# utiasASRL/dICP

Measured on AMD Instinct MI355X. Metric: ICP cloud-iterations/sec (fwd+bwd), B=256x16384-pt clouds per GPU, higher is better.
Workload: dtype f32

## Files before the change

### dicp_amd/_lib.py

```python
import ctypes
import os
import subprocess
import threading

_HERE = os.path.dirname(os.path.abspath(__file__))
_ROOT = os.path.dirname(_HERE)
LIB_PATH = os.environ.get("DICP_HIP_LIB") or os.path.join(_HERE, "libdicp_hip.so")
SOURCES = [os.path.join(_HERE, "csrc", f) for f in ("dicp_kernels.hip", "knn_f16.hip", "dicp_call.hip", "normals.hip", "voxel.hip", "knn_points.hip", "fps.hip", "ball_query.hip", "knn_grid.hip", "group.hip", "inverse.hip", "knn_det.hip", "normals_det.hip", "filter.hip")]
HEADERS = ([os.path.join(_HERE, "csrc", f) for f in ("dicp_math.h", "dicp_common.h", "dicp_internal.h", "dicp_fill.h", "dicp_normals.h", "dicp_voxel.h", "dicp_topk.h", "dicp_fps.h", "dicp_ball.h", "dicp_gridknn.h", "kernels_grid.h", "kernels_grid_plan.h", "dicp_group.h", "dicp_group_launch.h", "dicp_inverse.h", "dicp_knn_det.h", "kernels_normals.h", "dicp_normals_det.h", "dicp_filter.h")]
           + [os.path.join(_HERE, "csrc", "kernels_%s.h" % f) for f in ("setup", "search", "setup_sort", "rows", "accumulate", "backward", "soft_svd", "host")]
           + [os.path.join(_ROOT, "include", "dicp_hip.h")])

F32, F64 = 0, 1
PT2PT, PT2PL = 0, 1
LOSS_NONE, LOSS_HUBER, LOSS_CAUCHY, LOSS_TRIM = 0, 1, 2, 3
KNN_AUTO, KNN_VALU, KNN_MFMA, KNN_SWEEP, KNN_GUMBEL = 0, 1, 2, 3, 4
FPS_AUTO, FPS_RESIDENT, FPS_STREAMED = 0, 1, 2
POOL_SUM, POOL_MEAN, POOL_MAX = 0, 1, 2
NACC_PAD, NBWD_PAD, KAB_SAVE = 32, 16, 40
PAIR_SHARDS = 64
ABI_VERSION = 11
_ERRORS = {1: "null pointer", 2: "bad shape/stride", 3: "unsupported dtype", 4: "bad enum value", 5: "misaligned buffer"}

vp, i32, i64, f64 = ctypes.c_void_p, ctypes.c_int32, ctypes.c_int64, ctypes.c_double
# ... 152 lines not shown
    "dicp_accumulate_bwd_window": ([i32, ctypes.POINTER(WeightParams), vp, vp, i32, vp, vp, vp, vp, vp, vp, vp, vp, vp, i32, i32, i32, vp, vp, vp, vp, vp, i32, vp], ctypes.c_int),
    "dicp_resolve_matches": ([vp, vp, i32, vp, i32, i32, vp, vp], ctypes.c_int),
    "dicp_match_order_scratch_bytes": ([i32, i32, i32], ctypes.c_size_t),
    "dicp_match_order": ([i32, vp, vp, i32, i32, vp, ctypes.c_size_t, vp, vp], ctypes.c_int),
    "dicp_window_reduce": ([i32, vp, vp, vp, vp, vp, vp, i32, i32, i32, i32, i32, vp, i32, i32, vp], ctypes.c_int),
    "dicp_permute_add_rows": ([i32, vp, vp, i32, i32, i32, i32, i32, i32, vp, i32, i32, vp], ctypes.c_int),
    "dicp_pose_grad_in": ([i32, vp, vp, i32, vp], ctypes.c_int),
    "dicp_pose_grad_out": ([i32, vp, vp, i32, vp, i32, vp], ctypes.c_int),
    "dicp_permute_rows": ([i32, vp, vp, i32, i32, i32, i32, i32, i32, vp, i32, i32, vp], ctypes.c_int),
    "dicp_gather_rows": ([i32, vp, vp, i32, i32, i32, i32, vp, vp], ctypes.c_int),
    "dicp_scatter_add_rows": ([i32, vp, vp, i32, i32, i32, i32, vp, vp], ctypes.c_int),
    "dicp_pack_list": ([i32, vp, vp, vp, i32, i32, i32, vp, vp, vp], ctypes.c_int),
    "dicp_unpack_list": ([i32, vp, vp, vp, vp, i32, i32, i32, i32, vp], ctypes.c_int),
    "dicp_accumulate": ([i32, ctypes.POINTER(WeightParams), vp, vp, i32, vp, vp, vp, vp, vp, i32, i32, i32, vp, vp, i64, vp], ctypes.c_int),
    "dicp_step": ([i32, ctypes.POINTER(StepIO), i32, vp], ctypes.c_int),
    "dicp_icp_forward": ([i32, ctypes.POINTER(WeightParams), ctypes.POINTER(LoopBuffers), i32, i32, i32, i32, i32, f64, i32, i32, vp], ctypes.c_int),
    "dicp_icp_forward_plan": ([i32, ctypes.POINTER(WeightParams), ctypes.POINTER(LoopBuffers), ctypes.POINTER(SegmentPlan), i32, i32, i32, i32, i32, f64, vp], ctypes.c_int),
    "dicp_icp_backward": ([i32, ctypes.POINTER(WeightParams), ctypes.POINTER(LoopBuffers), i32, i32, i32, i32, vp, vp, i32, vp, vp, vp, vp, vp, vp, i32, i32, vp], ctypes.c_int),
    "dicp_step_bwd": ([i32, vp, vp, i32, i32, vp, vp, i64, vp, vp, vp, vp, i32, vp], ctypes.c_int),
    "dicp_accumulate_bwd": ([i32, ctypes.POINTER(WeightParams), vp, vp, i32, vp, vp, vp, vp, vp, vp, vp, i32, i32, i32, vp, vp, vp, vp, vp], ctypes.c_int),
    "dicp_gumbel_nn": ([i32, vp, vp, i32, vp, ctypes.c_uint32, f64, f64, i32, i32, i32, vp, vp, vp], ctypes.c_int),
    "dicp_gumbel_nn_bwd": ([i32, vp, vp, i32, vp, ctypes.c_uint32, f64, f64, vp, vp, vp, i32, i32, i32, vp, vp, vp], ctypes.c_int),
    "dicp_kabsch_accumulate": ([i32, vp, vp, i32, vp, vp, vp, i32, f64, vp, i32, i32, i32, vp, vp], ctypes.c_int),
    "dicp_kabsch_step": ([i32, vp, i32, vp, vp, vp, i32, vp], ctypes.c_int),
    "dicp_kabsch_step_bwd": ([i32, vp, vp, vp, i32, vp], ctypes.c_int),
    "dicp_kabsch_forward": ([i32, ctypes.POINTER(KabschBuffers), i32, i32, i32, i32, f64, i32, f64, i32, i32, vp], ctypes.c_int),
    "dicp_kabsch_bwd": ([i32, vp, vp, i32, vp, vp, vp, i32, f64, vp, vp, i32, i32, i32, vp, vp, vp, vp], ctypes.c_int),
    "dicp_transform_points": ([i32, vp, vp, vp, i32, i32, vp], ctypes.c_int),
    "dicp_transform_points_bwd": ([i32, vp, vp, vp, vp, vp, i32, i32, vp], ctypes.c_int),
    "dicp_loss_weight": ([i32, i32, i32, f64, f64, vp, i64, i32, vp, vp], ctypes.c_int),
    "dicp_loss_weight_bwd": ([i32, i32, i32, f64, f64, vp, vp, i64, i32, vp, vp], ctypes.c_int),
    "dicp_call_plan": ([i32, ctypes.POINTER(Call), ctypes.POINTER(CallLayout)], ctypes.c_int),
    "dicp_call_forward": ([i32, ctypes.POINTER(WeightParams), ctypes.POINTER(Call), vp], ctypes.c_int),
    "dicp_call_backward_plan": ([i32, ctypes.POINTER(WeightParams), ctypes.POINTER(Call), i32, i32, ctypes.POINTER(CallBackwardLayout)], ctypes.c_int),
# ... 133 lines not shown
```

### dicp_amd/csrc/dicp_kernels.hip

```cpp
#include <hip/hip_runtime.h>
#include <hip/hip_ext.h>
#include <stdint.h>

#include "dicp_common.h"
#include "dicp_internal.h"
#include "dicp_fill.h"

namespace {

#include "kernels_setup.h"
#include "kernels_search.h"
#include "kernels_setup_sort.h"
#include "kernels_rows.h"
#include "kernels_accumulate.h"
#include "kernels_backward.h"
#include "kernels_soft_svd.h"
#include "kernels_host.h"

}

extern "C" {

int dicp_abi_version(void) { return DICP_ABI_VERSION; }
int dicp_copy(void* dst, const void* src, size_t bytes, void* stream) {
// ... 403 lines not shown
            ps.nbr = (T*)ca->nbr; ps.gdirty = ca->gdirty; ps.pend = ca->pend; ps.cloud = ca->cloud; ps.fresh = ca->fresh; ps.units = ca->units; ps.sets = ca->sets; ps.scount = ca->scount; \
            if (P.mode == MODE_PT2PL) DICP_ACC(T, MODE_PT2PL, true, ps); else DICP_ACC(T, MODE_PT2PT, true, ps); \
        } else { if (P.mode == MODE_PT2PL) DICP_ACC(T, MODE_PT2PL, false, ps); else DICP_ACC(T, MODE_PT2PT, false, ps); } } while (0)
    if (dtype == DICP_F32) DICP_ACC_T(float); else DICP_ACC_T(double);
#undef DICP_ACC_T
#undef DICP_ACC
    return launch_status();
}

int dicp_accumulate(int dtype, const dicp_weight_params* prm, const void* src, const void* tgt, int c,
                    const int32_t* idx, const void* pose, const void* w_init, const void* alive, const int32_t* src_rows,
                    int N, int n, int m, void* partials, void* w_out, int64_t w_stride, void* stream) {
    return accumulate_go(dtype, prm, src, tgt, c, idx, pose, w_init, alive, src_rows, N, n, m, partials, w_out, w_stride, stream, nullptr);
}

int dicp_step(int dtype, const dicp_step_io* io, int N, void* stream) {
    if (!io || !io->partials || !io->pose_in || !io->pose_out || !io->delta || !io->cost || !io->alive || !io->alive_out ||
        !io->converged || !io->iterations || !io->matched_ratio || !io->n_start) return DICP_ERR_NULL;
    if (bad_dtype(dtype)) return DICP_ERR_DTYPE;
    if (N <= 0 || io->nblk <= 0 || (io->dim != 2 && io->dim != 3) || io->delta_stride < 6 || io->cost_stride < 1 ||
        (io->w_cur && io->w_stride < io->n)) return DICP_ERR_SHAPE;
    hipStream_t st = (hipStream_t)stream;
    begin_launch();
    if (dtype == DICP_F32) step_kernel<float><<<N, WAVE, 0, st>>>(*io, N);
    else                   step_kernel<double><<<N, WAVE, 0, st>>>(*io, N);
    return launch_status();
}

struct SkipHost { int32_t* skip; double* mref; const void* alive_k; int32_t* live_k; double eps; int k; };
static int step_bwd_go(int dtype, const double* gpose_in, const void* bwd_partials, int nblk, int dim,
                       const void* pose_k, const void* delta_k, int64_t delta_stride, const double* areg_k,
                       void* gs, void* gb, double* gpose_out, int N, void* stream, const SkipHost& sh) {
    if (!gpose_in || !pose_k || !delta_k || !areg_k || !gs || !gb || !gpose_out || (sh.skip && !sh.mref)) return DICP_ERR_NULL;
    if (bad_dtype(dtype)) return DICP_ERR_DTYPE;
    if (N <= 0 || (dim != 2 && dim != 3) || delta_stride < 6 || (bwd_partials && nblk <= 0)) return DICP_ERR_SHAPE;
    hipStream_t st = (hipStream_t)stream;
    begin_launch();
    if (dtype == DICP_F32)
        step_bwd_kernel<float><<<N, WAVE, 0, st>>>(gpose_in, (const float*)bwd_partials, nblk, dim, (const float*)pose_k,
                                                  (const float*)delta_k, (long)delta_stride, areg_k, (float*)gs, (float*)gb, gpose_out, N,
                                                  SkipArgs<float>{sh.skip, sh.mref, (const float*)sh.alive_k, sh.live_k, sh.eps, sh.k});
    else
        step_bwd_kernel<double><<<N, WAVE, 0, st>>>(gpose_in, (const double*)bwd_partials, nblk, dim, (const double*)pose_k,
                                                   (const double*)delta_k, (long)delta_stride, areg_k, (double*)gs, (double*)gb, gpose_out, N,
                                                   SkipArgs<double>{sh.skip, sh.mref, (const double*)sh.alive_k, sh.live_k, sh.eps, sh.k});
    return launch_status();
}
int dicp_step_bwd(int dtype, const double* gpose_in, const void* bwd_partials, int nblk, int dim,
                  const void* pose_k, const void* delta_k, int64_t delta_stride, const double* areg_k,
                  void* gs, void* gb, double* gpose_out, int N, void* stream) {
    return step_bwd_go(dtype, gpose_in, bwd_partials, nblk, dim, pose_k, delta_k, delta_stride, areg_k, gs, gb, gpose_out, N, stream, SkipHost{});
}

static int accumulate_bwd_go(int dtype, const dicp_weight_params* prm, const void* src, const void* tgt, int c,
                             const int32_t* idx, const void* pose, const void* w_init, const void* alive,
                             const void* gs, const void* gb, const int32_t* src_rows, int N, int n, int m,
                             void* gsrc, void* gtgt, void* gw, void* bwd_partials, void* stream, const int32_t* skip);
int dicp_accumulate_bwd(int dtype, const dicp_weight_params* prm, const void* src, const void* tgt, int c,
                        const int32_t* idx, const void* pose, const void* w_init, const void* alive,
                        const void* gs, const void* gb, const int32_t* src_rows, int N, int n, int m,
                        void* gsrc, void* gtgt, void* gw, void* bwd_partials, void* stream) {
    return accumulate_bwd_go(dtype, prm, src, tgt, c, idx, pose, w_init, alive, gs, gb, src_rows, N, n, m, gsrc, gtgt, gw, bwd_partials, stream, nullptr);
}
static int accumulate_bwd_go(int dtype, const dicp_weight_params* prm, const void* src, const void* tgt, int c,
                             const int32_t* idx, const void* pose, const void* w_init, const void* alive,
                             const void* gs, const void* gb, const int32_t* src_rows, int N, int n, int m,
// ... 652 lines not shown
```

### dicp_amd/csrc/dicp_math.h

```cpp
#pragma once
#include <math.h>

#if defined(__HIPCC__)
#define DICP_HD __host__ __device__ __forceinline__
#else
#define DICP_HD inline
#endif

namespace dicp {

enum Mode { MODE_PT2PT = 0, MODE_PT2PL = 1 };
enum Loss { LOSS_NONE = 0, LOSS_HUBER = 1, LOSS_CAUCHY = 2, LOSS_TRIM = 3 };

constexpr int ACC_A = 0, ACC_B = 21, ACC_COST = 27, ACC_SUMW = 28, ACC_NMATCH = 29, NACC = 30;
constexpr int NACC_PAD = 32;
constexpr int NBWD = 12, NBWD_PAD = 16;

struct WeightParams {
    int mode;
    int trim_on;
    int differentiable;
    int loss;
    double trim_dist;
    double tanh_k;
// ... 363 lines not shown
    for (int i = 0; i < D; ++i)
#pragma unroll
        for (int j = 0; j < D; ++j) Areg[i * 6 + j] = M[i * D + j];
    for (int i = 0; i < 6; ++i) delta6[i] = 0.0;
    if (solve_fixed<D>(M, rhs, x)) {
#pragma unroll
        for (int i = 0; i < D; ++i) delta6[i + OFF] = -x[i];
    }
}

DICP_HD void step_solve(const double* A6, const double* b6, int dim, double* delta6, double* Areg) {
    if (dim == 2) step_solve_fixed<3>(A6, b6, delta6, Areg);
    else          step_solve_fixed<6>(A6, b6, delta6, Areg);
}

DICP_HD void step_forward(const double* A6, const double* b6, int dim, const double* C, const double* r,
                          double* delta6, double* Cn, double* rn, double* Areg) {
    step_solve(A6, b6, dim, delta6, Areg);
    double R[9];
    so3_exp(delta6, R);
    for (int i = 0; i < 3; ++i)
        for (int j = 0; j < 3; ++j)
            Cn[i * 3 + j] = R[0 * 3 + i] * C[0 * 3 + j] + R[1 * 3 + i] * C[1 * 3 + j] + R[2 * 3 + i] * C[2 * 3 + j];
    for (int i = 0; i < 3; ++i) rn[i] = r[i] - delta6[3 + i];
}

template <int D>
DICP_HD void step_backward_fixed(const double* gCn, const double* grn, const double* C,
                                 const double* delta6, const double* Areg,
                                 double* Gs, double* gb, double* gC, double* gr) {
    constexpr int OFF = (D == 3) ? 2 : 0;
    double R[9];
    so3_exp(delta6, R);
    double gR[9];
    for (int i = 0; i < 3; ++i)
        for (int j = 0; j < 3; ++j) {
            gC[i * 3 + j] = R[i * 3 + 0] * gCn[0 * 3 + j] + R[i * 3 + 1] * gCn[1 * 3 + j] + R[i * 3 + 2] * gCn[2 * 3 + j];
            gR[i * 3 + j] = C[i * 3 + 0] * gCn[j * 3 + 0] + C[i * 3 + 1] * gCn[j * 3 + 1] + C[i * 3 + 2] * gCn[j * 3 + 2];
        }
    for (int i = 0; i < 3; ++i) gr[i] = grn[i];
    double Mm[9];
    for (int i = 0; i < 3; ++i)
        for (int j = 0; j < 3; ++j)
            Mm[i * 3 + j] = gR[i * 3 + 0] * R[j * 3 + 0] + gR[i * 3 + 1] * R[j * 3 + 1] + gR[i * 3 + 2] * R[j * 3 + 2];
    const double v[3] = {Mm[7] - Mm[5], Mm[2] - Mm[6], Mm[3] - Mm[1]};
    double a, b, c;
    so3_coeffs(delta6, a, b, c);
    const double* phi = delta6;
    const double pv = phi[0] * v[0] + phi[1] * v[1] + phi[2] * v[2];
    double pxv[3];
    cross3(phi, v, pxv);
    double gd[6];
    for (int i = 0; i < 3; ++i) gd[i] = a * v[i] + c * phi[i] * pv - b * pxv[i];
    for (int i = 0; i < 3; ++i) gd[3 + i] = -grn[i];
    double Mx[D * D], rhs[D], g[D];
#pragma unroll
    for (int i = 0; i < D; ++i) {
#pragma unroll
        for (int j = 0; j < D; ++j) Mx[i * D + j] = Areg[i * 6 + j];
        rhs[i] = gd[i + OFF];
    }
    for (int i = 0; i < 36; ++i) Gs[i] = 0.0;
    for (int i = 0; i < 6; ++i) gb[i] = 0.0;
    if (!solve_fixed<D>(Mx, rhs, g)) return;
#pragma unroll
    for (int i = 0; i < D; ++i) {
        gb[i + OFF] = -g[i];
#pragma unroll
        for (int j = 0; j < D; ++j) Gs[(i + OFF) * 6 + (j + OFF)] = -(g[i] * delta6[j + OFF] + delta6[i + OFF] * g[j]);
    }
}

DICP_HD void step_backward(const double* gCn, const double* grn, int dim, const double* C,
                           const double* delta6, const double* Areg,
                           double* Gs, double* gb, double* gC, double* gr) {
    if (dim == 2) step_backward_fixed<3>(gCn, grn, C, delta6, Areg, Gs, gb, gC, gr);
    else          step_backward_fixed<6>(gCn, grn, C, delta6, Areg, Gs, gb, gC, gr);
}

constexpr int KAB_S0 = 0, KAB_SP = 1, KAB_SY = 4, KAB_M = 7, KAB_PP = 16, KAB_YY = 17, NKAB = 18;
constexpr int KAB_SAVE = 40;

#define DICP_SVD3_ROTATE(p, q)                                                                                              \
    {                                                                                                                       \
        double a = 0, b = 0, g = 0;                                                                                         \
        _Pragma("unroll") for (int i = 0; i < 3; ++i) { a += G[i * 3 + p] * G[i * 3 + p]; b += G[i * 3 + q] * G[i * 3 + q]; g += G[i * 3 + p] * G[i * 3 + q]; } \
// ... 143 lines not shown
```

### dicp_amd/csrc/kernels_accumulate.h

```cpp
template <typename T, int H>
__device__ __forceinline__ void halve_step(T* v, int lane) {
    const bool up = (lane & (2 * H)) != 0;
#pragma unroll
    for (int k = 0; k < H; ++k) {
        const T keep = up ? v[H + k] : v[k];
        const T give = up ? v[k] : v[H + k];
        v[k] = keep + __shfl_xor(give, 2 * H);
    }
}
template <typename T, int NV, int PAD, int NT>
__device__ __forceinline__ void block_reduce_store(T* v, T* __restrict__ out, T* lds ) {
    static_assert(NV <= 32 && PAD >= NV, "reduce-scatter over 32 slots");
    const int tid = threadIdx.x, lane = tid & (WAVE - 1), wave = tid >> 6;
    if constexpr (NV <= 16) {
        T a[16];
#pragma unroll
        for (int k = 0; k < 16; ++k) a[k] = k < NV ? v[k] : T(0);
        halve_step<T, 8>(a, lane);
        halve_step<T, 4>(a, lane);
        halve_step<T, 2>(a, lane);
        halve_step<T, 1>(a, lane);
        T x = a[0] + __shfl_xor(a[0], 1);
        x += __shfl_xor(x, 32);
        const int slot = ((lane >> 4) & 1) * 8 + ((lane >> 3) & 1) * 4 + ((lane >> 2) & 1) * 2 + ((lane >> 1) & 1);
// ... 225 lines not shown
    io.cost_stride = B.K;
    io.areg = B.hist.areg ? B.hist.areg + (size_t)k * N * 36 : nullptr;
    io.alive = (const char*)B.hist.alive + (size_t)k * N * es; io.alive_out = (char*)B.hist.alive + (size_t)(k + 1) * N * es;
    io.converged = B.converged; io.iterations = B.iterations; io.matched_ratio = B.matched_ratio;
    io.n_start = B.n_start; io.n_matched = B.n_matched;
    io.w_cur = (char*)B.hist.w + (size_t)k * B.hist.w_iter * es;
    io.w_prev = k > k0 ? (const char*)B.hist.w + (size_t)(k - 1) * B.hist.w_iter * es : (const char*)B.hist.w_prev0; io.w_stride = B.hist.w_stride;
    io.n_not_converged = B.counters + k;
    io.rmax = B.cert.rmax; io.dcum = B.cert.dcum; io.dcum_stride = 2 * (B.K + 1);
    io.cert_cloud = B.cert.cloud;
    io.cert_qu = nullptr; io.cert_units = 0; io.glist_cap = 0; io.glist = nullptr; io.gcount = nullptr; io.cert_scount = nullptr; io.cert_slist = nullptr;
    io.w_copied = 0;
    return io;
}

template <typename T, int NT>
__device__ __forceinline__ void step_body(const dicp_step_io& io, int cloud, int tid) {
    __shared__ double sacc[NACC_PAD], sA[36], sAreg[36], spose[12], sout[24], smisc[16];
    __shared__ T sframe[12];
    __shared__ int scc[7];
    __shared__ int s_copy, s_next_state;
    __shared__ T s_dnext[2];
    if (tid < WAVE) {
        const int slot_i = tid & 31, part = tid >> 5;
        const T* pp = (const T*)io.partials + (size_t)cloud * io.nblk * NACC_PAD + slot_i;
        double s = 0.0;
        constexpr int UB = 8;
        for (int b0 = part; b0 < io.nblk; b0 += 2 * UB) {
            T v[UB];
#pragma unroll
            for (int u = 0; u < UB; ++u) v[u] = (b0 + 2 * u < io.nblk) ? pp[(size_t)(b0 + 2 * u) * NACC_PAD] : T(0);
#pragma unroll
            for (int u = 0; u < UB; ++u) if (b0 + 2 * u < io.nblk) s += (double)v[u];
        }
        s += __shfl_down(s, 32);
        if (tid < NACC_PAD) sacc[tid] = s;
        if (tid < 12) spose[tid] = (double)((const T*)io.pose_in)[(size_t)cloud * 12 + tid];
        if (tid == 40) smisc[0] = (double)((const T*)io.alive)[cloud];
        if (tid == 41) smisc[1] = io.cost_prev ? (double)((const T*)io.cost_prev)[(size_t)cloud * io.cost_stride] : 0.0;
        if (tid >= 42 && tid < 46) smisc[2 + (tid - 42)] = io.dcum ? (double)((const T*)io.rmax)[(size_t)cloud * 4 + (tid - 42)] : 0.0;
        if (tid >= 46 && tid < 49) smisc[6 + (tid - 46)] = io.frame ? (double)((const T*)io.frame)[(size_t)cloud * 12 + 9 + (tid - 46)] : 0.0;
        if (tid == 49) smisc[9] = io.dcum ? (double)((const T*)io.dcum)[(size_t)cloud * io.dcum_stride + 2 * io.iter] : 0.0;
        if (tid == 50) smisc[10] = (double)((const T*)io.n_start)[cloud];
        if (tid == 51) smisc[11] = (double)((const T*)io.iterations)[cloud];
        if (tid == 52) smisc[12] = (double)((const T*)io.matched_ratio)[cloud];
        if (tid >= 12 && tid < 24 && io.frame) sframe[tid - 12] = ((const T*)io.frame)[(size_t)cloud * 12 + (tid - 12)];
        if (tid >= 24 && tid < 31 && io.cert_cloud) scc[tid - 24] = io.cert_cloud[(size_t)cloud * CERT_CLOUD + (tid - 24)];
    }
    __syncthreads();
    if (tid == 0) {
        double* d6 = sout;
        unpack_sym6(sacc + ACC_A, sA);
        step_solve(sA, sacc + ACC_B, io.dim, d6, sAreg);
        T* dout = (T*)io.delta + (size_t)cloud * io.delta_stride;
        double nrm2 = 0.0;
        for (int k = 0; k < 6; ++k) { const T v = (T)d6[k]; dout[k] = v; d6[k] = (double)v; nrm2 += d6[k] * d6[k]; }
        double R[9];
        so3_exp(d6, R);
        T* pout = (T*)io.pose_out + (size_t)cloud * 12;
        const double* C = spose;
        T pn[12];
        for (int i = 0; i < 3; ++i)
            for (int j = 0; j < 3; ++j)
                pn[i * 3 + j] = (T)(R[0 * 3 + i] * C[0 * 3 + j] + R[1 * 3 + i] * C[1 * 3 + j] + R[2 * 3 + i] * C[2 * 3 + j]);
        for (int k = 0; k < 3; ++k) pn[9 + k] = (T)(spose[9 + k] - d6[3 + k]);
        for (int k = 0; k < 12; ++k) pout[k] = pn[k];
        if (io.dcum) {
            const double rad = smisc[2], p0[3] = {smisc[3], smisc[4], smisc[5]};
            double dC = 0.0, mv = 0.0, rn2 = 0.0;
            for (int i = 0; i < 3; ++i) {
                double m = (double)pn[9 + i] - spose[9 + i];
                for (int j = 0; j < 3; ++j) { const double d = (double)pn[i * 3 + j] - spose[i * 3 + j]; dC += d * d; m += d * p0[j]; }
                mv += m * m;
// ... 62 lines not shown
                if (costly || state > 0) cc[7] += 1;
                cc[0] = 0; cc[1] = 0; cc[3] = 0; cc[6] = 0;
            }
        }
    }
    __syncthreads();
    if (io.cert_qu && io.glist && tid < WAVE) {
        const T spent = cert_spent<T>(s_dnext);
        const int st = s_next_state;
        const bool certs_on = st <= 0 && st != CERT_RECERTIFY;
        const T* qu = (const T*)io.cert_qu + (size_t)cloud * io.cert_units;
        int32_t* list = io.glist + (size_t)(cloud & 7) * io.glist_cap;
        for (int u0 = 0; u0 < io.cert_units; u0 += WAVE) {
            const int u = u0 + tid;
            bool work = false;
            if (u < io.cert_units) { const T v = qu[u]; work = !(certs_on && v >= T(0) && v > spent); }
            const unsigned long long mk = __ballot(work);
            if (mk) {
                int base = 0;
                if (tid == 0) base = atomicAdd(io.gcount + (cloud & 7), __popcll(mk));
                base = __shfl(base, 0);
                const int rank = __builtin_amdgcn_mbcnt_hi((unsigned)(mk >> 32), __builtin_amdgcn_mbcnt_lo((unsigned)mk, 0u));
                if (work && base + rank < io.glist_cap) list[base + rank] = cloud * io.cert_units + u;
            }
        }
        if (io.cert_scount) {
            if (!certs_on) { if (tid == 0) io.cert_scount[cloud] = 0; }
            else {
                const int nwr = (io.n + WAVE - 1) / WAVE;
                const int have = min(io.cert_scount[cloud], io.n);
                const int nch = (have + WAVE - 1) / WAVE;
                if (io.cert_slist && nch > 0) {
                    const int upto = min(nch * WAVE, io.n);
                    for (int e = have + tid; e < upto; e += WAVE) io.cert_slist[(size_t)cloud * io.n + e] = -1;
                    if (tid == 0 && upto > have) io.cert_scount[cloud] = upto;
                }
                if (nch > 0) {
                    int base = 0;
                    if (tid == 0) base = atomicAdd(io.gcount + (cloud & 7), nch);
                    base = __shfl(base, 0);
                    for (int c = tid; c < nch; c += WAVE)
                        if (base + c < io.glist_cap) list[base + c] = -1 - (cloud * nwr + c);
                }
            }
        }
    }
    if (io.areg && tid < 36) io.areg[(size_t)cloud * 36 + tid] = sAreg[tid];
    if (s_copy) {
        T* wc = (T*)io.w_cur + (size_t)cloud * io.w_stride;
        const T* wp = (const T*)io.w_prev + (size_t)cloud * io.w_stride;
        for (int i = tid; i < io.n; i += NT) wc[i] = wp[i];
    }
}

template <typename T>
__global__ __launch_bounds__(WAVE) void step_kernel(dicp_step_io io, int N) {
    step_body<T, WAVE>(io, blockIdx.x, threadIdx.x);
}

__global__ __launch_bounds__(WAVE) void counters_report_kernel(const int32_t* __restrict__ counters, int32_t* __restrict__ host, int k0, int cnt, int tag) {
    for (int k = threadIdx.x; k < cnt; k += WAVE) {
        const int v = __hip_atomic_load(counters + k0 + k, __ATOMIC_RELAXED, __HIP_MEMORY_SCOPE_AGENT);
        __hip_atomic_store(host + k0 + k, (tag & 0x7ff00000) | (v < 0xfffff ? v : 0xfffff), __ATOMIC_RELAXED, __HIP_MEMORY_SCOPE_SYSTEM);
    }
}

template <typename T, int MODE>
__global__ __launch_bounds__(BLOCK) void icp_small_forward_kernel(WeightParams P, dicp_loop_buffers B, int N, int n, int m, int dim,
                                                                  int const_iter, double tolerance, int k0, int k1) {
    using T4 = typename V4<T>::type;
    extern __shared__ __align__(32) unsigned char small_lds[];
    T4* tg = reinterpret_cast<T4*>(small_lds);
// ... 65 lines not shown
```

### dicp_amd/csrc/kernels_backward.h

```cpp
template <typename T, int MODE>
__global__ __launch_bounds__(BLOCK) void accumulate_bwd_kernel(WeightParams P, const T* __restrict__ src, const T* __restrict__ tgt, int c,
                                                               const int32_t* __restrict__ idx, const T* __restrict__ pose,
                                                               const T* __restrict__ w_init, const T* __restrict__ alive,
                                                               const T* __restrict__ gs, const T* __restrict__ gb,
                                                               int N, int n, int m, int bpc,
                                                               T* __restrict__ gsrc, T* __restrict__ gtgt, T* __restrict__ gw,
                                                               T* __restrict__ bwd_partials, const int32_t* __restrict__ src_rows,
                                                               const int32_t* __restrict__ skip ) {
    constexpr int CV = (MODE == MODE_PT2PL) ? 6 : 3;
    __shared__ T red[(BLOCK / WAVE) * NBWD_PAD];
    __shared__ T stage_v[(BLOCK / WAVE) * WAVE * CV];
    __shared__ int stage_j[BLOCK];
    int cloud, blk;
    if (!decode_block(bpc, N, cloud, blk)) return;
    if (skip && skip[cloud]) {
        if (threadIdx.x < NBWD_PAD) bwd_partials[((size_t)cloud * bpc + blk) * NBWD_PAD + threadIdx.x] = T(0);
        return;
    }
    const int tid = threadIdx.x, lane = tid & (WAVE - 1), wave = tid >> 6;
    T C[9], r[3], Gs[36], Gb[6];
    load_pose(pose, cloud, C, r);
#pragma unroll
    for (int k = 0; k < 36; ++k) Gs[k] = gs[(size_t)cloud * 36 + k];
#pragma unroll
// ... 475 lines not shown
    if (!nan && 16.0 * worst <= sk.eps * ref) return 2;
    if (!nan && m > ref) sk.mref[cloud] = m;
    if (sk.live_k) atomicAdd(sk.live_k, 1);
    return 0;
}

DICP_HD void pose_pass_through(const double* gCn, const double* grn, const double* delta6, double* gC, double* gr) {
    double R[9];
    so3_exp(delta6, R);
    for (int i = 0; i < 3; ++i)
        for (int j = 0; j < 3; ++j)
            gC[i * 3 + j] = R[i * 3 + 0] * gCn[0 * 3 + j] + R[i * 3 + 1] * gCn[1 * 3 + j] + R[i * 3 + 2] * gCn[2 * 3 + j];
    for (int i = 0; i < 3; ++i) gr[i] = grn[i];
}

template <typename T>
__global__ __launch_bounds__(WAVE) void step_bwd_kernel(const double* __restrict__ gpose_in, const T* __restrict__ bwd_partials,
                                                        int nblk, int dim, const T* __restrict__ pose_k,
                                                        const T* __restrict__ delta_k, long delta_stride,
                                                        const double* __restrict__ areg_k, T* __restrict__ gs,
                                                        T* __restrict__ gb, double* __restrict__ gpose_out, int N, SkipArgs<T> sk) {
    __shared__ double sg[NBWD_PAD], sC[9], sd[6], sAreg[36], sGs[36], sGb[6], sgo[12], sdmax[6], smref;
    __shared__ int salive, sended;
    const int cloud = blockIdx.x, tid = threadIdx.x;
    if (sk.skip) {
        double dm[6] = {0.0, 0.0, 0.0, 0.0, 0.0, 0.0};
        for (int j = 1 + tid; j <= sk.k; j += WAVE) {
            const T* dp = delta_k + (size_t)cloud * delta_stride - (size_t)j * 6;
#pragma unroll
            for (int i = 0; i < 6; ++i) { const double v = fabs((double)dp[i]); dm[i] = max_or_nan(v, dm[i]); }
        }
#pragma unroll
        for (int i = 0; i < 6; ++i) {
#pragma unroll
            for (int off = WAVE / 2; off > 0; off >>= 1) { const double o = __shfl_down(dm[i], off); dm[i] = max_or_nan(o, dm[i]); }
        }
// ... 28 lines not shown
    }
    __syncthreads();
    if (sended) {
        if (tid == 0) {
            double g[12], d[6], go[12];
#pragma unroll
            for (int k = 0; k < 12; ++k) g[k] = sg[k];
#pragma unroll
            for (int k = 0; k < 6; ++k) d[k] = sd[k];
            pose_pass_through(g, g + 9, d, go, go + 9);
#pragma unroll
            for (int k = 0; k < 12; ++k) gpose_out[(size_t)cloud * 12 + k] = go[k];
        }
        return;
    }
    if (tid == 0) {
        double g[12], C[9], d[6], A[36], Gs[36], Gb[6], go[12];
#pragma unroll
        for (int k = 0; k < 12; ++k) g[k] = sg[k];
#pragma unroll
        for (int k = 0; k < 9; ++k) C[k] = sC[k];
#pragma unroll
        for (int k = 0; k < 6; ++k) d[k] = sd[k];
#pragma unroll
        for (int k = 0; k < 36; ++k) A[k] = sAreg[k];
        step_backward(g, g + 9, dim, C, d, A, Gs, Gb, go, go + 9);
#pragma unroll
        for (int k = 0; k < 36; ++k) sGs[k] = Gs[k];
#pragma unroll
        for (int k = 0; k < 6; ++k) sGb[k] = Gb[k];
#pragma unroll
        for (int k = 0; k < 12; ++k) sgo[k] = go[k];
    }
    __syncthreads();
    if (sk.skip) {
        const int D = dim == 2 ? 3 : 6, OFF = dim == 2 ? 2 : 0;
        double v = 0.0, vb = 0.0, va = 0.0;
        if (tid < 36) {
            const int i = tid / 6, j = tid - 6 * i;
            if (i < D && j < D) v = fabs(sGs[(i + OFF) * 6 + (j + OFF)]) * sqrt(fabs(sAreg[i * 6 + i])) * sqrt(fabs(sAreg[j * 6 + j]));
        } else if (tid < 42) {
// ... 12 lines not shown
            if (!salive) verdict = 1;
            else {
                const double worst = gmax * amp > m ? gmax * amp : m;
                if (!nan && 16.0 * worst <= sk.eps * smref) verdict = 2;
                else {
                    if (!nan && m > smref) sk.mref[cloud] = m;
                    if (sk.live_k) atomicAdd(sk.live_k, 1);
                }
            }
            sk.skip[cloud] = verdict;
        }
    }
    if (tid < 36) gs[(size_t)cloud * 36 + tid] = (T)sGs[tid];
    if (tid < 6) gb[(size_t)cloud * 6 + tid] = (T)sGb[tid];
    if (tid < 12) gpose_out[(size_t)cloud * 12 + tid] = sgo[tid];
}

template <typename T, int MODE>
__global__ __launch_bounds__(BLOCK) void icp_small_backward_kernel(WeightParams P, dicp_loop_buffers B, int N, int n, int m, int dim,
                                                                   const double* __restrict__ gpose_in, double* __restrict__ gpose_out,
                                                                   int have_partials, T* __restrict__ gsrc, T* __restrict__ gtgt,
                                                                   T* __restrict__ gw, T* __restrict__ bwd_partials, int nblk, int k0, int k1) {
    constexpr int CV = (MODE == MODE_PT2PL) ? 6 : 3;
    extern __shared__ __align__(16) unsigned char small_bwd_lds[];
    T* gt = reinterpret_cast<T*>(small_bwd_lds);
    __shared__ double sg[NBWD_PAD], sC[9], sd[6], sAreg[36], sGs[36], sGb[6], sgo[12], spart[NBWD_PAD], sdmax[6], sR[WAVE * 9];
    constexpr int NT = BLOCK;
    __shared__ T red[(NT / WAVE) * NBWD_PAD];
    __shared__ T part[NBWD_PAD];
    __shared__ int s_skip;
// ... 335 lines not shown
```

### include/dicp_hip.h

```cpp
#ifndef DICP_HIP_H
#define DICP_HIP_H
#include <stddef.h>
#include <stdint.h>

#ifdef __cplusplus
extern "C" {
#endif

#define DICP_ABI_VERSION 11

enum { DICP_F32 = 0, DICP_F64 = 1 };
enum { DICP_PT2PT = 0, DICP_PT2PL = 1 };
enum { DICP_LOSS_NONE = 0, DICP_LOSS_HUBER = 1, DICP_LOSS_CAUCHY = 2, DICP_LOSS_TRIM = 3 };
enum { DICP_KNN_AUTO = 0, DICP_KNN_VALU = 1, DICP_KNN_MFMA = 2, DICP_KNN_SWEEP = 3 ,
       DICP_KNN_GUMBEL = 4  };
enum { DICP_ERR_NULL = 1, DICP_ERR_SHAPE = 2, DICP_ERR_DTYPE = 3, DICP_ERR_ENUM = 4, DICP_ERR_ALIGN = 5, DICP_ERR_ABI = 6  };

#define DICP_NACC_PAD 32
#define DICP_NBWD_PAD 16

typedef struct dicp_weight_params {
    int32_t mode;
    int32_t trim_on;
    int32_t differentiable;
// ... 89 lines not shown
    const void* rmax;
    void* dcum;
    int64_t dcum_stride;
    int32_t* cert_cloud;
    const void* cert_qu;
    int32_t cert_units;
    int32_t glist_cap;
    int32_t* glist;
    int32_t* gcount;
    int32_t* cert_scount;
    int32_t* cert_slist;
    int32_t w_copied;
} dicp_step_io;

int dicp_step(int dtype, const dicp_step_io* io, int N, void* stream);

typedef struct dicp_gumbel_loop {
    const void* const* U;
    const uint32_t* seeds;
    double eps, tau;
    void* ps_t;
    void* nbr;
    void* lse;
    void* g_nbr;
    void* g_ps;
} dicp_gumbel_loop;

typedef struct dicp_search_buffers {
    int32_t knn_variant;
    int32_t m_pad;
// ... 119 lines not shown
} dicp_segment_plan;
int dicp_icp_forward_plan(int dtype, const dicp_weight_params* prm, const dicp_loop_buffers* buf, const dicp_segment_plan* plan, int N, int n, int m,
                          int dim, int const_iter, double tolerance, void* stream);
int dicp_icp_backward(int dtype, const dicp_weight_params* prm, const dicp_loop_buffers* buf, int N, int n, int m, int dim,
                      double* gpose, double* gpose_tmp, int have_partials, void* gs, void* gb, void* gsrc, void* gtgt, void* gw,
                      void* bwd_partials, int k0, int k1, void* stream);
int dicp_resolve_matches(const int32_t* spos, const int32_t* spos_of, int k, const int32_t* src_rows ,
                         int N, int n, int32_t* out, void* stream);
size_t dicp_match_order_scratch_bytes(int dtype, int N, int n);
int dicp_match_order(int dtype, const int32_t* spos_ref, const int32_t* src_rows, int N, int n, void* scratch, size_t scratch_bytes, int32_t* qorder, void* stream);


int dicp_step_bwd(int dtype, const double* gpose_in, const void* bwd_partials, int nblk, int dim,
                  const void* pose_k, const void* delta_k, int64_t delta_stride, const double* areg_k,
                  void* gs, void* gb, double* gpose_out, int N, void* stream);

int dicp_accumulate_bwd(int dtype, const dicp_weight_params* prm, const void* src, const void* tgt, int c,
                        const int32_t* idx, const void* pose, const void* w_init, const void* alive,
                        const void* gs, const void* gb, const int32_t* src_rows, int N, int n, int m,
                        void* gsrc, void* gtgt, void* gw, void* bwd_partials, void* stream);

int dicp_window_blocks(int dtype, int n, int m_pad);
int dicp_window_rows(int dtype);
int dicp_bwd_tail_max_blocks(int dtype);
int dicp_accumulate_bwd_window(int dtype, const dicp_weight_params* prm, const void* src_s, const void* tgt_s, int c,
                               const int32_t* spos, const int32_t* spos_ref, const int32_t* qorder, const void* pose, const void* w_s,
                               const void* alive, const void* gs, const void* gb, const int32_t* src_rows, int N, int n, int m_pad, void* gsrc_s, void* slab,
                               void* gts_far, void* gw_s, void* bwd_partials, int overwrite, void* stream);
int dicp_window_reduce(int dtype, const void* slab, const int32_t* spos_ref, const int32_t* qorder, const int32_t* tperm, const void* gts_far,
                       const int32_t* src_rows, int N, int n, int m, int m_pad, int cv, void* gtgt, int c, int overwrite, void* stream);
// ... 278 lines not shown
```

Before: 3.288 million.

## Solve per-cloud 6x6 step systems cooperatively across a wavefront

Replaces the single-thread Gaussian elimination in the forward step and backward step kernels with a wave-wide solve: the augmented matrix is spread one element per lane (8x8 grid), with pivot search via readlane and row updates via shuffles. The step kernel also prefetches the first cert unit and set count during the initial load phase, so later per-thread global reads are avoided. Serial variants are kept as separately exported entry points. The per-cloud step is latency bound with 63 of 64 lanes idle, so this targets that serial tail, at the cost of extra shuffles and slightly different floating-point rounding.

```diff
diff --git a/dicp_amd/_lib.py b/dicp_amd/_lib.py
--- a/dicp_amd/_lib.py
+++ b/dicp_amd/_lib.py
@@ -190,10 +190,12 @@
     "dicp_unpack_list": ([i32, vp, vp, vp, vp, i32, i32, i32, i32, vp], ctypes.c_int),
     "dicp_accumulate": ([i32, ctypes.POINTER(WeightParams), vp, vp, i32, vp, vp, vp, vp, vp, i32, i32, i32, vp, vp, i64, vp], ctypes.c_int),
     "dicp_step": ([i32, ctypes.POINTER(StepIO), i32, vp], ctypes.c_int),
+    "dicp_step_serial": ([i32, ctypes.POINTER(StepIO), i32, vp], ctypes.c_int),
     "dicp_icp_forward": ([i32, ctypes.POINTER(WeightParams), ctypes.POINTER(LoopBuffers), i32, i32, i32, i32, i32, f64, i32, i32, vp], ctypes.c_int),
     "dicp_icp_forward_plan": ([i32, ctypes.POINTER(WeightParams), ctypes.POINTER(LoopBuffers), ctypes.POINTER(SegmentPlan), i32, i32, i32, i32, i32, f64, vp], ctypes.c_int),
     "dicp_icp_backward": ([i32, ctypes.POINTER(WeightParams), ctypes.POINTER(LoopBuffers), i32, i32, i32, i32, vp, vp, i32, vp, vp, vp, vp, vp, vp, i32, i32, vp], ctypes.c_int),
     "dicp_step_bwd": ([i32, vp, vp, i32, i32, vp, vp, i64, vp, vp, vp, vp, i32, vp], ctypes.c_int),
+    "dicp_step_bwd_serial": ([i32, vp, vp, i32, i32, vp, vp, i64, vp, vp, vp, vp, i32, vp], ctypes.c_int),
     "dicp_accumulate_bwd": ([i32, ctypes.POINTER(WeightParams), vp, vp, i32, vp, vp, vp, vp, vp, vp, vp, i32, i32, i32, vp, vp, vp, vp, vp], ctypes.c_int),
     "dicp_gumbel_nn": ([i32, vp, vp, i32, vp, ctypes.c_uint32, f64, f64, i32, i32, i32, vp, vp, vp], ctypes.c_int),
     "dicp_gumbel_nn_bwd": ([i32, vp, vp, i32, vp, ctypes.c_uint32, f64, f64, vp, vp, vp, i32, i32, i32, vp, vp, vp], ctypes.c_int),
diff --git a/dicp_amd/csrc/dicp_kernels.hip b/dicp_amd/csrc/dicp_kernels.hip
--- a/dicp_amd/csrc/dicp_kernels.hip
+++ b/dicp_amd/csrc/dicp_kernels.hip
@@ -441,7 +441,7 @@
     return accumulate_go(dtype, prm, src, tgt, c, idx, pose, w_init, alive, src_rows, N, n, m, partials, w_out, w_stride, stream, nullptr);
 }
 
-int dicp_step(int dtype, const dicp_step_io* io, int N, void* stream) {
+static int step_go(int dtype, const dicp_step_io* io, int N, void* stream, bool lanes) {
     if (!io || !io->partials || !io->pose_in || !io->pose_out || !io->delta || !io->cost || !io->alive || !io->alive_out ||
         !io->converged || !io->iterations || !io->matched_ratio || !io->n_start) return DICP_ERR_NULL;
     if (bad_dtype(dtype)) return DICP_ERR_DTYPE;
@@ -449,21 +449,37 @@
         (io->w_cur && io->w_stride < io->n)) return DICP_ERR_SHAPE;
     hipStream_t st = (hipStream_t)stream;
     begin_launch();
-    if (dtype == DICP_F32) step_kernel<float><<<N, WAVE, 0, st>>>(*io, N);
-    else                   step_kernel<double><<<N, WAVE, 0, st>>>(*io, N);
-    return launch_status();
-}
+    if (!lanes) {
+        if (dtype == DICP_F32) step_serial_kernel<float><<<N, WAVE, 0, st>>>(*io, N);
+        else                   step_serial_kernel<double><<<N, WAVE, 0, st>>>(*io, N);
+    }
+    else if (dtype == DICP_F32) step_kernel<float><<<N, WAVE, 0, st>>>(*io, N);
+    else                        step_kernel<double><<<N, WAVE, 0, st>>>(*io, N);
+    return launch_status();
+}
+int dicp_step(int dtype, const dicp_step_io* io, int N, void* stream) { return step_go(dtype, io, N, stream, true); }
+int dicp_step_serial(int dtype, const dicp_step_io* io, int N, void* stream) { return step_go(dtype, io, N, stream, false); }
 
 struct SkipHost { int32_t* skip; double* mref; const void* alive_k; int32_t* live_k; double eps; int k; };
 static int step_bwd_go(int dtype, const double* gpose_in, const void* bwd_partials, int nblk, int dim,
                        const void* pose_k, const void* delta_k, int64_t delta_stride, const double* areg_k,
-                       void* gs, void* gb, double* gpose_out, int N, void* stream, const SkipHost& sh) {
+                       void* gs, void* gb, double* gpose_out, int N, void* stream, const SkipHost& sh, bool lanes = true) {
     if (!gpose_in || !pose_k || !delta_k || !areg_k || !gs || !gb || !gpose_out || (sh.skip && !sh.mref)) return DICP_ERR_NULL;
     if (bad_dtype(dtype)) return DICP_ERR_DTYPE;
     if (N <= 0 || (dim != 2 && dim != 3) || delta_stride < 6 || (bwd_partials && nblk <= 0)) return DICP_ERR_SHAPE;
     hipStream_t st = (hipStream_t)stream;
     begin_launch();
-    if (dtype == DICP_F32)
+    if (!lanes) {
+        if (dtype == DICP_F32)
+            step_bwd_serial_kernel<float><<<N, WAVE, 0, st>>>(gpose_in, (const float*)bwd_partials, nblk, dim, (const float*)pose_k,
+                                                             (const float*)delta_k, (long)delta_stride, areg_k, (float*)gs, (float*)gb, gpose_out, N,
+                                                             SkipArgs<float>{sh.skip, sh.mref, (const float*)sh.alive_k, sh.live_k, sh.eps, sh.k});
+        else
+            step_bwd_serial_kernel<double><<<N, WAVE, 0, st>>>(gpose_in, (const double*)bwd_partials, nblk, dim, (const double*)pose_k,
+                                                              (const double*)delta_k, (long)delta_stride, areg_k, (double*)gs, (double*)gb, gpose_out, N,
+                                                              SkipArgs<double>{sh.skip, sh.mref, (const double*)sh.alive_k, sh.live_k, sh.eps, sh.k});
+    }
+    else if (dtype == DICP_F32)
         step_bwd_kernel<float><<<N, WAVE, 0, st>>>(gpose_in, (const float*)bwd_partials, nblk, dim, (const float*)pose_k,
                                                   (const float*)delta_k, (long)delta_stride, areg_k, (float*)gs, (float*)gb, gpose_out, N,
                                                   SkipArgs<float>{sh.skip, sh.mref, (const float*)sh.alive_k, sh.live_k, sh.eps, sh.k});
@@ -477,6 +493,11 @@
                   const void* pose_k, const void* delta_k, int64_t delta_stride, const double* areg_k,
                   void* gs, void* gb, double* gpose_out, int N, void* stream) {
     return step_bwd_go(dtype, gpose_in, bwd_partials, nblk, dim, pose_k, delta_k, delta_stride, areg_k, gs, gb, gpose_out, N, stream, SkipHost{});
+}
+int dicp_step_bwd_serial(int dtype, const double* gpose_in, const void* bwd_partials, int nblk, int dim,
+                         const void* pose_k, const void* delta_k, int64_t delta_stride, const double* areg_k,
+                         void* gs, void* gb, double* gpose_out, int N, void* stream) {
+    return step_bwd_go(dtype, gpose_in, bwd_partials, nblk, dim, pose_k, delta_k, delta_stride, areg_k, gs, gb, gpose_out, N, stream, SkipHost{}, false);
 }
 
 static int accumulate_bwd_go(int dtype, const dicp_weight_params* prm, const void* src, const void* tgt, int c,
diff --git a/dicp_amd/csrc/dicp_math.h b/dicp_amd/csrc/dicp_math.h
--- a/dicp_amd/csrc/dicp_math.h
+++ b/dicp_amd/csrc/dicp_math.h
@@ -401,6 +401,71 @@
     else          step_solve_fixed<6>(A6, b6, delta6, Areg);
 }
 
+#if defined(__HIPCC__)
+__device__ __forceinline__ double lane_read(double v, int src) {
+    const int lo = __builtin_amdgcn_readlane(__double2loint(v), src), hi = __builtin_amdgcn_readlane(__double2hiint(v), src);
+    return __hiloint2double(hi, lo);
+}
+template <int D>
+__device__ __forceinline__ bool wave_solve_fixed(double m, int lane, double (&x)[D]) {
+    const int r = lane >> 3, c = lane & 7;
+#pragma unroll
+    for (int k = 0; k < D; ++k) {
+        int piv = k;
+        double pv = lane_read(m, k * 8 + k), best = fabs(pv);
+#pragma unroll
+        for (int i = k + 1; i < D; ++i) {
+            const double e = lane_read(m, i * 8 + k), v = fabs(e);
+            if (v > best) { best = v; piv = i; pv = e; }
+        }
+        if (best == 0.0) return false;
+        const int from = (r == k) ? piv : ((r == piv) ? k : r);
+        const double mine = __shfl(m, from * 8 + k), pk = __shfl(m, piv * 8 + c);
+        m = __shfl(m, from * 8 + c);
+        const double inv = 1.0 / pv;
+        const double f = mine * inv;
+        if (r > k && r < D && c > k && c <= D) m = fma(-f, pk, m);
+    }
+    double U[D][D + 1];
+#pragma unroll
+    for (int i = 0; i < D; ++i)
+#pragma unroll
+        for (int cc = i; cc <= D; ++cc) U[i][cc] = lane_read(m, i * 8 + cc);
+#pragma unroll
+    for (int i = D - 1; i >= 0; --i) {
+        double v = U[i][D];
+#pragma unroll
+        for (int cc = i + 1; cc < D; ++cc) v = fma(-U[i][cc], x[cc], v);
+        x[i] = v / U[i][i];
+    }
+    return true;
+}
+
+__device__ __forceinline__ void wave_step_solve(const double* acc, int dim, int lane, double* areg_out, double (&delta6)[6]) {
+    const int D = ndof(dim), OFF = slot(dim, 0);
+    const int r = lane >> 3, c = lane & 7;
+    double m = 0.0;
+    if (r < D && c < D) {
+        const int a = r + OFF, b = c + OFF;
+        m = acc[ACC_A + (a <= b ? tri(a, b) : tri(b, a))];
+        if (r == c) m += 1e-12;
+    } else if (r < D && c == D) m = acc[ACC_B + r + OFF];
+    if (areg_out && r < 6 && c < 6) areg_out[r * 6 + c] = (r < D && c < D) ? m : 0.0;
+#pragma unroll
+    for (int i = 0; i < 6; ++i) delta6[i] = 0.0;
+    if (dim == 2) {
+        double x[3];
+        if (wave_solve_fixed<3>(m, lane, x)) { delta6[2] = -x[0]; delta6[3] = -x[1]; delta6[4] = -x[2]; }
+    } else {
+        double x[6];
+        if (wave_solve_fixed<6>(m, lane, x)) {
+#pragma unroll
+            for (int i = 0; i < 6; ++i) delta6[i] = -x[i];
+        }
+    }
+}
+#endif
+
 DICP_HD void step_forward(const double* A6, const double* b6, int dim, const double* C, const double* r,
                           double* delta6, double* Cn, double* rn, double* Areg) {
     step_solve(A6, b6, dim, delta6, Areg);
@@ -412,11 +477,7 @@
     for (int i = 0; i < 3; ++i) rn[i] = r[i] - delta6[3 + i];
 }
 
-template <int D>
-DICP_HD void step_backward_fixed(const double* gCn, const double* grn, const double* C,
-                                 const double* delta6, const double* Areg,
-                                 double* Gs, double* gb, double* gC, double* gr) {
-    constexpr int OFF = (D == 3) ? 2 : 0;
+DICP_HD void step_backward_head(const double* gCn, const double* grn, const double* C, const double* delta6, double* gC, double* gr, double* gd) {
     double R[9];
     so3_exp(delta6, R);
     double gR[9];
@@ -437,9 +498,16 @@
     const double pv = phi[0] * v[0] + phi[1] * v[1] + phi[2] * v[2];
     double pxv[3];
     cross3(phi, v, pxv);
-    double gd[6];
     for (int i = 0; i < 3; ++i) gd[i] = a * v[i] + c * phi[i] * pv - b * pxv[i];
     for (int i = 0; i < 3; ++i) gd[3 + i] = -grn[i];
+}
+template <int D>
+DICP_HD void step_backward_fixed(const double* gCn, const double* grn, const double* C,
+                                 const double* delta6, const double* Areg,
+                                 double* Gs, double* gb, double* gC, double* gr) {
+    constexpr int OFF = (D == 3) ? 2 : 0;
+    double gd[6];
+    step_backward_head(gCn, grn, C, delta6, gC, gr, gd);
     double Mx[D * D], rhs[D], g[D];
 #pragma unroll
     for (int i = 0; i < D; ++i) {
@@ -457,6 +525,30 @@
         for (int j = 0; j < D; ++j) Gs[(i + OFF) * 6 + (j + OFF)] = -(g[i] * delta6[j + OFF] + delta6[i + OFF] * g[j]);
     }
 }
+
+#if defined(__HIPCC__)
+template <int D>
+__device__ __forceinline__ void wave_step_backward_fixed(const double (&gd)[6], const double* delta6, const double* Areg, int lane, double& gs_t, double& gb_t) {
+    constexpr int OFF = (D == 3) ? 2 : 0;
+    const int r = lane >> 3, c = lane & 7;
+    double m = 0.0;
+    if (r < D && c < D) m = Areg[r * 6 + c];
+    else if (r < D && c == D) {
+#pragma unroll
+        for (int i = 0; i < D; ++i) if (r == i) m = gd[i + OFF];
+    }
+    double g[D];
+    const bool ok = wave_solve_fixed<D>(m, lane, g);
+    gs_t = 0.0; gb_t = 0.0;
+    if (!ok) return;
+    const int a = (lane < 36 ? lane / 6 : 0) - OFF, b = (lane < 36 ? lane % 6 : 0) - OFF;
+    double ga = 0.0, gb_ = 0.0, gl = 0.0;
+#pragma unroll
+    for (int i = 0; i < D; ++i) { if (a == i) ga = g[i]; if (b == i) gb_ = g[i]; if (lane - OFF == i) gl = g[i]; }
+    if (lane < 36 && a >= 0 && a < D && b >= 0 && b < D) gs_t = -(ga * delta6[b + OFF] + delta6[a + OFF] * gb_);
+    if (lane - OFF >= 0 && lane - OFF < D) gb_t = -gl;
+}
+#endif
 
 DICP_HD void step_backward(const double* gCn, const double* grn, int dim, const double* C,
                            const double* delta6, const double* Areg,
diff --git a/dicp_amd/csrc/kernels_accumulate.h b/dicp_amd/csrc/kernels_accumulate.h
--- a/dicp_amd/csrc/kernels_accumulate.h
+++ b/dicp_amd/csrc/kernels_accumulate.h
@@ -263,13 +263,15 @@
     return io;
 }
 
-template <typename T, int NT>
+template <typename T, int NT, bool LANES = true>
 __device__ __forceinline__ void step_body(const dicp_step_io& io, int cloud, int tid) {
     __shared__ double sacc[NACC_PAD], sA[36], sAreg[36], spose[12], sout[24], smisc[16];
     __shared__ T sframe[12];
     __shared__ int scc[7];
     __shared__ int s_copy, s_next_state;
     __shared__ T s_dnext[2];
+    T qu_first = T(0);
+    int sets_have = 0;
     if (tid < WAVE) {
         const int slot_i = tid & 31, part = tid >> 5;
         const T* pp = (const T*)io.partials + (size_t)cloud * io.nblk * NACC_PAD + slot_i;
@@ -295,17 +297,41 @@
         if (tid == 52) smisc[12] = (double)((const T*)io.matched_ratio)[cloud];
         if (tid >= 12 && tid < 24 && io.frame) sframe[tid - 12] = ((const T*)io.frame)[(size_t)cloud * 12 + (tid - 12)];
         if (tid >= 24 && tid < 31 && io.cert_cloud) scc[tid - 24] = io.cert_cloud[(size_t)cloud * CERT_CLOUD + (tid - 24)];
+        if (LANES && io.cert_qu && io.glist) {
+            if (tid < io.cert_units) qu_first = ((const T*)io.cert_qu)[(size_t)cloud * io.cert_units + tid];
+            if (io.cert_scount) sets_have = io.cert_scount[cloud];
+        }
     }
     __syncthreads();
+#if defined(DICP_STEP_ABLATE)
+    constexpr bool SOLVE_LANES = false;
+#else
+    constexpr bool SOLVE_LANES = LANES;
+#endif
+    double dl[6];
+    if (SOLVE_LANES && tid < WAVE) wave_step_solve(sacc, io.dim, tid, io.areg ? io.areg + (size_t)cloud * 36 : nullptr, dl);
     if (tid == 0) {
         double* d6 = sout;
-        unpack_sym6(sacc + ACC_A, sA);
-        step_solve(sA, sacc + ACC_B, io.dim, d6, sAreg);
+        if (SOLVE_LANES) {
+            for (int k = 0; k < 6; ++k) d6[k] = dl[k];
+        } else {
+            unpack_sym6(sacc + ACC_A, sA);
+#if defined(DICP_STEP_ABLATE)
+            for (int k = 0; k < 36; ++k) sAreg[k] = sA[k];
+            for (int k = 0; k < 6; ++k) d6[k] = 1e-3 + 0.0 * sacc[ACC_B + k];
+#else
+            step_solve(sA, sacc + ACC_B, io.dim, d6, sAreg);
+#endif
+        }
         T* dout = (T*)io.delta + (size_t)cloud * io.delta_stride;
         double nrm2 = 0.0;
         for (int k = 0; k < 6; ++k) { const T v = (T)d6[k]; dout[k] = v; d6[k] = (double)v; nrm2 += d6[k] * d6[k]; }
         double R[9];
+#if defined(DICP_STEP_ABLATE)
+        for (int k = 0; k < 9; ++k) R[k] = (k % 4 == 0) ? 1.0 : 0.0;
+#else
         so3_exp(d6, R);
+#endif
         T* pout = (T*)io.pose_out + (size_t)cloud * 12;
         const double* C = spose;
         T pn[12];
@@ -398,7 +424,7 @@
         for (int u0 = 0; u0 < io.cert_units; u0 += WAVE) {
             const int u = u0 + tid;
             bool work = false;
-            if (u < io.cert_units) { const T v = qu[u]; work = !(certs_on && v >= T(0) && v > spent); }
+            if (u < io.cert_units) { const T v = (LANES && u0 == 0) ? qu_first : qu[u]; work = !(certs_on && v >= T(0) && v > spent); }
             const unsigned long long mk = __ballot(work);
             if (mk) {
                 int base = 0;
@@ -412,7 +438,7 @@
             if (!certs_on) { if (tid == 0) io.cert_scount[cloud] = 0; }
             else {
                 const int nwr = (io.n + WAVE - 1) / WAVE;
-                const int have = min(io.cert_scount[cloud], io.n);
+                const int have = min(LANES ? sets_have : io.cert_scount[cloud], io.n);
                 const int nch = (have + WAVE - 1) / WAVE;
                 if (io.cert_slist && nch > 0) {
                     const int upto = min(nch * WAVE, io.n);
@@ -429,7 +455,7 @@
             }
         }
     }
-    if (io.areg && tid < 36) io.areg[(size_t)cloud * 36 + tid] = sAreg[tid];
+    if (!SOLVE_LANES && io.areg && tid < 36) io.areg[(size_t)cloud * 36 + tid] = sAreg[tid];
     if (s_copy) {
         T* wc = (T*)io.w_cur + (size_t)cloud * io.w_stride;
         const T* wp = (const T*)io.w_prev + (size_t)cloud * io.w_stride;
@@ -440,6 +466,10 @@
 template <typename T>
 __global__ __launch_bounds__(WAVE) void step_kernel(dicp_step_io io, int N) {
     step_body<T, WAVE>(io, blockIdx.x, threadIdx.x);
+}
+template <typename T>
+__global__ __launch_bounds__(WAVE) void step_serial_kernel(dicp_step_io io, int N) {
+    step_body<T, WAVE, false>(io, blockIdx.x, threadIdx.x);
 }
 
 __global__ __launch_bounds__(WAVE) void counters_report_kernel(const int32_t* __restrict__ counters, int32_t* __restrict__ host, int k0, int cnt, int tag) {
diff --git a/dicp_amd/csrc/kernels_backward.h b/dicp_amd/csrc/kernels_backward.h
--- a/dicp_amd/csrc/kernels_backward.h
+++ b/dicp_amd/csrc/kernels_backward.h
@@ -513,12 +513,12 @@
     for (int i = 0; i < 3; ++i) gr[i] = grn[i];
 }
 
-template <typename T>
-__global__ __launch_bounds__(WAVE) void step_bwd_kernel(const double* __restrict__ gpose_in, const T* __restrict__ bwd_partials,
-                                                        int nblk, int dim, const T* __restrict__ pose_k,
-                                                        const T* __restrict__ delta_k, long delta_stride,
-                                                        const double* __restrict__ areg_k, T* __restrict__ gs,
-                                                        T* __restrict__ gb, double* __restrict__ gpose_out, int N, SkipArgs<T> sk) {
+template <typename T, bool LANES>
+__device__ __forceinline__ void step_bwd_body(const double* __restrict__ gpose_in, const T* __restrict__ bwd_partials,
+                                              int nblk, int dim, const T* __restrict__ pose_k,
+                                              const T* __restrict__ delta_k, long delta_stride,
+                                              const double* __restrict__ areg_k, T* __restrict__ gs,
+                                              T* __restrict__ gb, double* __restrict__ gpose_out, int N, const SkipArgs<T>& sk) {
     __shared__ double sg[NBWD_PAD], sC[9], sd[6], sAreg[36], sGs[36], sGb[6], sgo[12], sdmax[6], smref;
     __shared__ int salive, sended;
     const int cloud = blockIdx.x, tid = threadIdx.x;
@@ -577,6 +577,27 @@
         }
         return;
     }
+#if !defined(DICP_STEP_ABLATE)
+    if (LANES) {
+        double g[12], C[9], d[6], gd[6], go[12];
+#pragma unroll
+        for (int k = 0; k < 12; ++k) g[k] = sg[k];
+#pragma unroll
+        for (int k = 0; k < 9; ++k) C[k] = sC[k];
+#pragma unroll
+        for (int k = 0; k < 6; ++k) d[k] = sd[k];
+        step_backward_head(g, g + 9, C, d, go, go + 9, gd);
+        double gs_t, gb_t;
+        if (dim == 2) wave_step_backward_fixed<3>(gd, sd, sAreg, tid, gs_t, gb_t);
+        else          wave_step_backward_fixed<6>(gd, sd, sAreg, tid, gs_t, gb_t);
+        if (tid < 36) sGs[tid] = gs_t;
+        if (tid < 6) sGb[tid] = gb_t;
+        if (tid == 0) {
+#pragma unroll
+            for (int k = 0; k < 12; ++k) sgo[k] = go[k];
+        }
+    } else
+#endif
     if (tid == 0) {
         double g[12], C[9], d[6], A[36], Gs[36], Gb[6], go[12];
 #pragma unroll
@@ -587,7 +608,13 @@
         for (int k = 0; k < 6; ++k) d[k] = sd[k];
 #pragma unroll
         for (int k = 0; k < 36; ++k) A[k] = sAreg[k];
+#if defined(DICP_STEP_ABLATE)
+        for (int k = 0; k < 36; ++k) Gs[k] = 1.0 + 0.0 * (A[k] + C[k % 9] + d[k % 6]);
+        for (int k = 0; k < 6; ++k) Gb[k] = 1.0;
+        for (int k = 0; k < 12; ++k) go[k] = g[k];
+#else
         step_backward(g, g + 9, dim, C, d, A, Gs, Gb, go, go + 9);
+#endif
 #pragma unroll
         for (int k = 0; k < 36; ++k) sGs[k] = Gs[k];
 #pragma unroll
@@ -630,6 +657,20 @@
     if (tid < 36) gs[(size_t)cloud * 36 + tid] = (T)sGs[tid];
     if (tid < 6) gb[(size_t)cloud * 6 + tid] = (T)sGb[tid];
     if (tid < 12) gpose_out[(size_t)cloud * 12 + tid] = sgo[tid];
+}
+template <typename T>
+__global__ __launch_bounds__(WAVE) void step_bwd_kernel(const double* __restrict__ gpose_in, const T* __restrict__ bwd_partials, int nblk, int dim,
+                                                        const T* __restrict__ pose_k, const T* __restrict__ delta_k, long delta_stride,
+                                                        const double* __restrict__ areg_k, T* __restrict__ gs, T* __restrict__ gb,
+                                                        double* __restrict__ gpose_out, int N, SkipArgs<T> sk) {
+    step_bwd_body<T, true>(gpose_in, bwd_partials, nblk, dim, pose_k, delta_k, delta_stride, areg_k, gs, gb, gpose_out, N, sk);
+}
+template <typename T>
+__global__ __launch_bounds__(WAVE) void step_bwd_serial_kernel(const double* __restrict__ gpose_in, const T* __restrict__ bwd_partials, int nblk, int dim,
+                                                               const T* __restrict__ pose_k, const T* __restrict__ delta_k, long delta_stride,
+                                                               const double* __restrict__ areg_k, T* __restrict__ gs, T* __restrict__ gb,
+                                                               double* __restrict__ gpose_out, int N, SkipArgs<T> sk) {
+    step_bwd_body<T, false>(gpose_in, bwd_partials, nblk, dim, pose_k, delta_k, delta_stride, areg_k, gs, gb, gpose_out, N, sk);
 }
 
 template <typename T, int MODE>
diff --git a/include/dicp_hip.h b/include/dicp_hip.h
--- a/include/dicp_hip.h
+++ b/include/dicp_hip.h
@@ -127,6 +127,7 @@
 } dicp_step_io;
 
 int dicp_step(int dtype, const dicp_step_io* io, int N, void* stream);
+int dicp_step_serial(int dtype, const dicp_step_io* io, int N, void* stream);
 
 typedef struct dicp_gumbel_loop {
     const void* const* U;
@@ -276,6 +277,9 @@
 int dicp_step_bwd(int dtype, const double* gpose_in, const void* bwd_partials, int nblk, int dim,
                   const void* pose_k, const void* delta_k, int64_t delta_stride, const double* areg_k,
                   void* gs, void* gb, double* gpose_out, int N, void* stream);
+int dicp_step_bwd_serial(int dtype, const double* gpose_in, const void* bwd_partials, int nblk, int dim,
+                         const void* pose_k, const void* delta_k, int64_t delta_stride, const double* areg_k,
+                         void* gs, void* gb, double* gpose_out, int N, void* stream);
 
 int dicp_accumulate_bwd(int dtype, const dicp_weight_params* prm, const void* src, const void* tgt, int c,
                         const int32_t* idx, const void* pose, const void* w_init, const void* alive,
```

After: 3.308 million (median of 6 runs). Within noise of the previous version (+0.6%).
